# Roco-scientist/NGS-Barcode-Count

Measured on AMD Instinct MI355X. Metric: reads/sec (whole node), 3x8nt DEL vs 3x1k refs, higher is better.
Workload: dtype u8

## Files before the change

### ngs-barcode-count_amd/csrc/bc_engine.hip

```cpp
#include <hip/hip_runtime.h>
#include <string.h>
#include <stdio.h>
#include <stdlib.h>
#include <unistd.h>

#include <algorithm>
#include <functional>
#include <thread>
#include <unordered_map>
#include <string>
#include <vector>

#include "../../include/barcode_count_hip.h"
#include "bc_kernel.h"
#include "bc_engine_impl.h"
#include "bc_fold.h"
#include "bc_synth.h"

extern "C" int bc_internal_table_pack_u8(const void* d_table_u32, const void* d_bits, uint64_t n, void* d_out_u8, void* d_ovf_idx_u64,
                                         void* d_ovf_val_u32, uint64_t ovf_capacity, uint64_t* n_ovf, int device_id, void* hip_stream);

namespace bc {

template <int NW, int NWW>
// ... 609 lines not shown
  if (const char* ch = getenv("BC_COUNT_LOG_HOT")) e->log_hot = atoi(ch) != 0;
  if (const char* cd = getenv("BC_COUNT_LOG_DEFER_RESET")) e->defer_reset = atoi(cd) != 0;
  if (const char* cf = getenv("BC_COUNT_LOG_FRESH")) e->fold_fresh = atoi(cf) != 0;
  if (const char* cm = getenv("BC_COUNT_LOG_MIN_READS")) e->log_min_reads = strtoull(cm, nullptr, 0);
  if (const char* cc = getenv("BC_COUNT_LOG_CHUNK")) {
    const uint64_t c = strtoull(cc, nullptr, 0) & ~63ull;
    if (c) e->log_chunk = std::min<uint64_t>(c, 1ull << 27);
  }
  if (P.lhash_vec) {
    const int rc = upload(e, e->h.lhash.data(), e->h.lhash.size() * 4, &P.lhash_a);
    if (rc) return rc;
  }
#ifdef BC_EXPERIMENT
  if (const char* pm = getenv("BC_PIPE")) e->pipe = atoi(pm) != 0;
#endif
  HIP_TRY(hipMalloc((void**)&e->d_plan, sizeof(DevPlan)));
  HIP_TRY(hipMemcpy(e->d_plan, &P, sizeof(DevPlan), hipMemcpyHostToDevice));
  for (uint32_t g = 0; g < P.n_groups; ++g) {
    const DevGroup& G = P.groups[g];
    if (G.mode != kSetDirect) continue;
    const uint32_t nq = 1u << (2 * G.len);
    hipLaunchKernelGGL(build_dtable_kernel, dim3((nq + 255) / 256), dim3(256), 0, e->stream, e->d_plan, g,
                       reinterpret_cast<uint32_t*>((uintptr_t)G.dtable_a));
    HIP_TRY(hipGetLastError());
  }
  if (P.sparse) {
    if (table_mem) {
      set_error("bc_engine_create: the plan keeps raw captures (no dense table); pass table_mem = NULL");
      return BC_ERR_INVALID;
    }
// ... 149 lines not shown
  int rc = settle_table_on(e, e->reset_stream);
  if (rc == BC_OK && !bits_stay_owed) rc = settle_bits_on(e, e->reset_stream);
  if (hipEventRecord(e->reset_join, e->reset_stream) != hipSuccess) {
    HIP_TRY(hipStreamSynchronize(e->reset_stream));
    return rc;
  }
  *join = true;
  return rc;
}

template <int NW, int NWW>
static int launch_match(bc_engine* e, const void* d_seq, const void* d_qual, const void* d_lens, const void* d_qlens, uint32_t stride,
                        uint32_t read_len, uint32_t nd, uint64_t n_reads, uint64_t trace_off, const MatchShape& s) {
  const bool use_log = log_mode_for(e, n_reads);
  const bool hot_on = !use_log || e->log_hot;
  const bool table_untouched = use_log && !hot_on && !e->h.plan.defer_search();
  const OwedPlan owed = owed_plan(e, use_log, table_untouched);
  if (owed.table == kOwedMain) {
    const int rc = settle_table_on(e, e->stream);
    if (rc != BC_OK) return rc;
  }
  if (owed.bits == kOwedMain) {
    const int rc = settle_bits_on(e, e->stream);
    if (rc != BC_OK) return rc;
  }
  const uint32_t flags = (e->pipe ? 1u : 0u) | (s.tables_generic ? 2u : 0u) | (s.hot_generic && hot_on ? 4u : 0u);
  if (s.lds + 64 > e->lds_limit) {
    set_error("read stride too large for one LDS tile");
    return BC_ERR_UNSUPPORTED;
  }
  auto kern = match_count_kernel<NW, NWW>;
  if (s.lds > 48 * 1024) HIP_TRY(hipFuncSetAttribute((const void*)kern, hipFuncAttributeMaxDynamicSharedMemorySize, (int)s.lds));
  int per_cu = 0;
  HIP_TRY(hipOccupancyMaxActiveBlocksPerMultiprocessor(&per_cu, (const void*)kern, kTPB, s.lds));
  if (per_cu < 1) per_cu = 1;
  const uint64_t resident = (uint64_t)per_cu * e->n_cus;
  const uint64_t blocks = std::min<uint64_t>((n_reads + kTPB - 1) / kTPB, resident);
  uint64_t blocks_jit = blocks;
  hipEvent_t e0 = nullptr, e1 = nullptr;
  if (e->timing) {
    HIP_TRY(hipEventCreate(&e0));
    HIP_TRY(hipEventCreate(&e1));
    HIP_TRY(hipEventRecord(e0, e->stream));
  }
  hipFunction_t jit_fn = nullptr;
  e->reads_seen += n_reads;
  if (NW <= 8 && NWW <= 4 && e->jit_mode != 0) {
    int per_cu_jit = 1;
    jit_fn = e->jit.function(e->h.plan, e->device, e->jit_mode, e->reads_seen, s, &per_cu_jit);
    if (jit_fn) blocks_jit = std::min<uint64_t>((n_reads + kTPB - 1) / kTPB, (uint64_t)per_cu_jit * e->n_cus);
  }
  if (use_log) {
    const int rc = ensure_log(e, std::min<uint64_t>(n_reads, e->log_chunk));
    if (rc != BC_OK) return rc;
  }
  const uint64_t chunk = use_log ? e->log_chunk : n_reads;
  bool join = false;
  if (use_log) {
    const int rc = fork_owed(e, owed, &join);
    if (rc != BC_OK) {
      if (join) (void)hipStreamWaitEvent(e->stream, e->reset_join, 0);
      (void)settle_owed(e);
      return rc;
    }
  }
// ... 9 lines not shown
    const uint8_t* a_seq = (const uint8_t*)d_seq + c0 * stride;
    const uint8_t* a_qual = d_qual ? (const uint8_t*)d_qual + c0 * stride : nullptr;
    const uint16_t* a_lens = d_lens ? (const uint16_t*)d_lens + c0 : nullptr;
    const uint16_t* a_qlens = d_qlens ? (const uint16_t*)d_qlens + c0 : nullptr;
    uint8_t* a_to = e->trace_outcome ? e->trace_outcome + trace_off + c0 : nullptr;
    uint64_t* a_ti = e->trace_idx ? e->trace_idx + trace_off + c0 : nullptr;
    uint32_t* a_log = use_log ? e->d_log : nullptr;
    uint64_t a_n = n_c;
    if (jit_fn) {
      uint32_t a_region = s.region;
      uint64_t a_smask = e->n_slots ? e->n_slots - 1 : 0;
      uint32_t a_flags = (e->pipe ? 1u : 0u) | (s.tables_jit ? 2u : 0u) | (s.hot_jit && hot_on ? 4u : 0u);
      void* args[] = {&a_seq, &a_qual, &a_lens, &a_qlens, &stride, &read_len, &nd, &a_n, &a_region, &e->d_table, &e->d_bits, &e->d_slots,
                      &e->d_vals, &a_smask, &e->d_counters, &a_to, &a_ti, &a_flags, &a_log};
      const uint64_t grid = std::min<uint64_t>(blocks_jit, (n_c + kTPB - 1) / kTPB);
      HIP_TRY(hipModuleLaunchKernel(jit_fn, (uint32_t)grid, 1, 1, kTPB, 1, 1, s.lds_jit, e->stream, args, nullptr));
    } else {
      const uint64_t grid = std::min<uint64_t>(blocks, (n_c + kTPB - 1) / kTPB);
      hipLaunchKernelGGL(kern, dim3((uint32_t)grid), dim3(kTPB), s.lds, e->stream, e->d_plan, a_seq, a_qual, a_lens, a_qlens, stride, read_len,
                         nd, a_n, s.region, e->d_table, e->d_bits, e->d_slots, e->d_vals, e->n_slots ? e->n_slots - 1 : 0, e->d_counters,
                         a_to, a_ti, flags, a_log);
    }
    HIP_TRY(hipGetLastError());
    if (use_log) {
      if (join) {
        HIP_TRY(hipStreamWaitEvent(e->stream, e->reset_join, 0));
        join = false;
      }
      const bool fresh = e->owed_bits;
      const int rc = fold_log(e, n_c, fresh);
      if (rc != BC_OK) return rc;
      e->owed_bits = false;
    }
  }
  if (e->d_bits) {
    e->bits_dirty = true;
    e->reads_since_fold += n_reads;
  }
  e->last_kernel = std::string(jit_fn ? "bc_jit_match_count<" : "match_count_kernel<") +
                   std::to_string(jit_fn ? s.jit.NW : NW) + "," + std::to_string(jit_fn ? s.jit.NWW : NWW) + ">";
  if (e->timing) {
    HIP_TRY(hipEventRecord(e1, e->stream));
    e->events.emplace_back(e0, e1);
  }
  return BC_OK;
}

static int ensure_long(bc_engine* e) {
  if (e->long_ready) return BC_OK;
  if (!e->long_only && !e->src_plan->lower_long(e->lh)) return BC_ERR_UNSUPPORTED;
  LongPlan& Q = e->lh.plan;
  int rc;
  if ((rc = upload(e, e->lh.const_pos.data(), e->lh.const_pos.size() * 4, &Q.const_pos_a))) return rc;
  if ((rc = upload(e, e->lh.const_chr.data(), e->lh.const_chr.size(), &Q.const_chr_a))) return rc;
  if ((rc = upload(e, e->lh.fmtn_pos.data(), e->lh.fmtn_pos.size() * 4, &Q.fmtn_pos_a))) return rc;
// ... 104 lines not shown
  const uint32_t maxlen = d_lens ? stride : read_len;
  if (maxlen > stride) {
    set_error("submit: read_len exceeds stride");
    return BC_ERR_INVALID;
  }
  const uint32_t nd = (maxlen + 3) / 4;
  HIP_TRY(hipSetDevice(e->device));
  e->table_materialized = false;
  counts_changed(e);
  {
    const int rc = set_reserve(e, n_reads);
    if (rc != BC_OK) return rc;
  }
  if (e->long_only || maxlen > 320u) return launch_long(e, d_seq, d_qual, d_lens, d_qlens, stride, read_len, n_reads, trace_off);
  const MatchShape s = match_shape(e->h.plan, e->table_entries, stride, read_len, d_lens != nullptr, e->trace_outcome != nullptr,
                                   e->lds_limit, e->pipe, e->lhash_mode);
  const int nww = s.jit.NWW;
#define BC_LAUNCH(NW_, NWW_) \
  return launch_match<NW_, NWW_>(e, d_seq, d_qual, d_lens, d_qlens, stride, read_len, nd, n_reads, trace_off, s)
  if (s.generic_nw == 4) {
    if (nww <= 1) BC_LAUNCH(4, 1);
    if (nww <= 2) BC_LAUNCH(4, 2);
    BC_LAUNCH(4, 4);
  }
  if (s.generic_nw == 8) {
    if (nww <= 2) BC_LAUNCH(8, 2);
    if (nww <= 4) BC_LAUNCH(8, 4);
    BC_LAUNCH(8, 8);
  }
  if (nww <= 4) BC_LAUNCH(10, 4);
  BC_LAUNCH(10, 10);
// ... 979 lines not shown
  HIP_TRY(hipEventRecord(e0, 0));
  hipLaunchKernelGGL(atomic_probe_kernel, dim3(blocks), dim3(256), 0, 0, (uint32_t*)d_table_u32, entries, per, 2ull, 1u);
  HIP_TRY(hipEventRecord(e1, 0));
  hipLaunchKernelGGL(atomic_probe_kernel, dim3(blocks), dim3(256), 0, 0, (uint32_t*)d_table_u32, entries, per, 2ull, 0xFFFFFFFFu);
  HIP_TRY(hipGetLastError());
  HIP_TRY(hipDeviceSynchronize());
  float ms = 0.f;
  HIP_TRY(hipEventElapsedTime(&ms, e0, e1));
  (void)hipEventDestroy(e0);
  (void)hipEventDestroy(e1);
  if (ms > 0.f) *atomics_per_s = (double)blocks * 256.0 * per / (ms * 1e-3);
  return BC_OK;
}

const char* bc_engine_kernel_name(bc_engine* e) { return e ? e->last_kernel.c_str() : ""; }

int bc_engine_count_log_folds(const bc_engine* e, uint64_t* n) {
  *n = e->log_folds;
  return BC_OK;
}

int bc_engine_gz_blocks_inflated(const bc_engine* e, uint64_t* n) {
  *n = e->gz_blocks;
  return BC_OK;
}

int bc_engine_gz_segments_inflated(const bc_engine* e, uint64_t* n) {
  *n = e->gz_segments;
  return BC_OK;
}
// ... 314 lines not shown
```

### ngs-barcode-count_amd/csrc/bc_engine_impl.h

```cpp
#ifndef BC_ENGINE_IMPL_H
#define BC_ENGINE_IMPL_H

#include <hip/hip_runtime.h>
#include <stdint.h>

#include <string>
#include <utility>
#include <vector>

#include "../../include/barcode_count_hip.h"
#include "bc_enrich.h"
#include "bc_jit.h"
#include "bc_plan.hpp"

#define HIP_TRY(expr)                                                                      \
  do {                                                                                     \
    hipError_t _e = (expr);                                                                \
    if (_e != hipSuccess) {                                                                \
      bc::set_error(std::string(#expr) + ": " + hipGetErrorString(_e));                    \
      if (_e == hipErrorOutOfMemory) (void)hipGetLastError();  \
      return _e == hipErrorOutOfMemory ? BC_ERR_NOMEM : BC_ERR_HIP;                        \
    }                                                                                      \
  } while (0)

// ... 76 lines not shown
  std::vector<float> launch_ms;
  std::vector<uint64_t> row_idx;
  std::vector<uint32_t> row_cnt;
  static constexpr int kStages = 2;
  uint8_t* pin[kStages] = {nullptr, nullptr};
  uint8_t* dev[kStages] = {nullptr, nullptr};
  hipEvent_t copied[kStages] = {nullptr, nullptr};
  hipEvent_t consumed[kStages] = {nullptr, nullptr};
  size_t stage_bytes = 0;
  uint32_t lds_limit = 0;
  uint32_t n_cus = 0;
  bc::JitKernels jit;
  uint64_t reads_seen = 0;
  int jit_mode = 1;
  std::string last_kernel;
  bool pipe = true;
  int lhash_mode = 1;
  unsigned long long* d_slots = nullptr;
  uint32_t* d_vals = nullptr;
  uint64_t n_slots = 0;
  uint32_t key_words = 1;
  uint32_t* d_ready = nullptr;
  std::vector<uint64_t> row_wide;
  uint64_t key_bound = 0;
  bool long_only = false, long_ready = false;
  bc::LongHost lh;
  bc::LongPlan* d_long = nullptr;
  const bc_plan* src_plan = nullptr;
  bool render_pool_ready = false;
  uint32_t* d_label_off = nullptr;
  uint8_t* d_label_bytes = nullptr;
// ... 28 lines not shown
```

### ngs-barcode-count_amd/csrc/bc_jit.h

```cpp
#pragma once
#include <hip/hip_runtime.h>
#include <stdint.h>

#include <atomic>
#include <map>
#include <memory>
#include <string>
#include <thread>
#include <vector>

#include "bc_plan.hpp"

namespace bc {

struct PlanSetup {
  int lhash_mode = 1;
  uint64_t n_bit_words = 0;
  uint64_t dirty_bytes = 0;
};
PlanSetup plan_setup(HostDevPlan& h, bool long_only, bool own_table);

inline int generic_nw(uint32_t maxlen) { return maxlen <= 128 ? 4 : (maxlen <= 256 ? 8 : 10); }

struct JitShape {
  int NW, NWW;
  bool lens, tables, trace;
  uint32_t stride, read_len, region;
  bool conservative = false;
  int min_waves = 3;
};

struct MatchShape {
  int generic_nw;
  uint32_t region;
  uint32_t lds, lds_jit;
  bool tables_generic, tables_jit;
  bool hot_generic, hot_jit;
  JitShape jit;
  int first_min_waves;
  uint64_t key;
};
MatchShape match_shape(const DevPlan& P, uint64_t table_entries, uint32_t stride, uint32_t read_len, bool lens, bool trace,
                       uint32_t lds_limit, bool pipe, int lhash_mode);

struct JitKernels {
  struct Jit {
    enum { kIdle = 0, kCompiling = 1, kCodeReady = 2, kLoaded = 3, kFailed = -1 };
    std::atomic<int> state{kIdle};
    std::thread worker;
    std::vector<char> code;
    std::string log;
    hipModule_t mod = nullptr;
    hipFunction_t fn = nullptr;
    int per_cu = 0;
  };
  std::map<uint64_t, std::unique_ptr<Jit>> slots;

  JitKernels() = default;
  JitKernels(const JitKernels&) = delete;
  JitKernels& operator=(const JitKernels&) = delete;
  ~JitKernels();
  hipFunction_t function(const DevPlan& plan, int device, int mode, uint64_t reads_seen, const MatchShape& s, int* per_cu);
};

}
```

### ngs-barcode-count_amd/csrc/bc_jit.hip

```cpp
#include <hip/hip_runtime.h>
#include <hip/hiprtc.h>
#include <dlfcn.h>
#include <errno.h>
#include <fcntl.h>
#include <spawn.h>
#include <stdio.h>
#include <stdlib.h>
#include <string.h>
#include <sys/stat.h>
#include <sys/wait.h>
#include <unistd.h>

#include <algorithm>

#include "../../include/barcode_count_hip.h"
#include "bc_jit.h"
#include "bc_kernel.h"

#include "bc_jit_sources.inc"

extern char** environ;

namespace bc {

// ... 72 lines not shown
#endif
  return ps;
}

static constexpr uint32_t kGfx950LdsBytes = 160u * 1024u;

static int jit_first_min_waves(int NW, uint32_t lds_per_wg, uint32_t lds_limit) {
#ifdef BC_EXPERIMENT
  if (const char* v = getenv("BC_JIT_MIN_WAVES")) return atoi(v);
#endif
  if (NW > 4) return 2;
  const int by_lds = (int)(lds_limit / (lds_per_wg + 64u));
  return std::max(3, std::min(5, by_lds));
}

MatchShape match_shape(const DevPlan& P, uint64_t table_entries, uint32_t stride, uint32_t read_len, bool lens, bool trace,
                       uint32_t lds_limit, bool pipe, int lhash_mode) {
  MatchShape s;
  const uint32_t maxlen = lens ? stride : read_len;
  s.generic_nw = generic_nw(maxlen);
  const uint32_t slack = (uint32_t)s.generic_nw * 32u + 16u + (P.L > stride ? P.L - stride : 0u);
  s.region = (64u * stride + slack + 15u) & ~15u;
  const uint32_t lds_tiles = s.region * (kTPB / 64) * ((P.quality_on && pipe) ? 2u : 1u) +
                             (P.defer_search() ? (kTPB / 64) * kQueueBytes : 0u);
  const uint32_t lds_tables = P.lhash_vec * 16u;
  const bool tables_fit = lds_tables != 0 && 2u * (lds_tiles + lds_tables + 64u) <= lds_limit;
  s.tables_generic = lhash_mode >= 2 && tables_fit;
  s.tables_jit = lhash_mode >= 1 && tables_fit;
#ifdef BC_NO_HOT
  const bool hot_ok = false;
#else
  const bool hot_ok = !P.sparse && !P.has_random && table_entries != 0 && table_entries <= 0xFFFFFFFFull;
#endif
  const uint32_t lds_generic = lds_tiles + (s.tables_generic ? lds_tables : 0u);
  const uint32_t lds_jit = lds_tiles + (s.tables_jit ? lds_tables : 0u);
  const auto hot_fits = [&](uint32_t lds) { return hot_ok && 2u * (lds + kHotBytes + 64u) <= lds_limit; };
  s.hot_generic = hot_fits(lds_generic);
  s.hot_jit = hot_fits(lds_jit);
  s.lds = lds_generic + (s.hot_generic ? kHotBytes : 0u);
  s.lds_jit = lds_jit + (s.hot_jit ? kHotBytes : 0u);
  JitShape& sh = s.jit;
  sh.NW = (int)((maxlen + 31) / 32);
  sh.NWW = maxlen >= P.L ? (int)((maxlen - P.L + 1 + 31) / 32) : 1;
  sh.lens = lens;
  sh.tables = s.tables_jit;
  sh.trace = trace;
  sh.stride = stride;
  sh.read_len = lens ? 0u : read_len;
  sh.region = s.region;
  s.first_min_waves = jit_first_min_waves(sh.NW, s.lds_jit, lds_limit);
  s.key = ((uint64_t)stride << 32) | ((uint64_t)sh.read_len << 16) |
          (uint64_t)(((sh.NW * 16 + sh.NWW) * 2 + (lens ? 1 : 0)) * 4 + (sh.tables ? 2 : 0) + (trace ? 1 : 0));
  return s;
}

static int code_scratch_bytes(const std::vector<char>& code) {
  static const char kKey[] = ".private_segment_fixed_size";
  const size_t kl = sizeof(kKey) - 1;
  if (code.size() < kl + 5) return -1;
  for (size_t i = 0; i + kl + 5 <= code.size(); ++i) {
    if (code[i] != '.' || memcmp(&code[i], kKey, kl) != 0) continue;
    const unsigned char* v = reinterpret_cast<const unsigned char*>(&code[i + kl]);
    if (v[0] < 0x80) return v[0];
    if (v[0] == 0xcc) return v[1];
    if (v[0] == 0xcd) return (v[1] << 8) | v[2];
    if (v[0] == 0xce) return (int)(((uint32_t)v[1] << 24) | (v[2] << 16) | (v[3] << 8) | v[4]);
// ... 3 lines not shown
}

static void push_flags(std::vector<std::string>& d, const char* flags) {
  std::string t;
  for (const char* c = flags;; ++c) {
    if (*c == ' ' || *c == ';' || *c == 0) {
      if (!t.empty()) d.push_back(t);
      t.clear();
      if (*c == 0) break;
    } else {
      t += *c;
    }
  }
}

static std::vector<std::string> jit_defines(int NW, int NWW, bool lens, bool tables, bool trace, uint32_t stride, uint32_t read_len,
                                            uint32_t region, bool conservative, int min_waves) {
  std::vector<std::string> d = {"-DJIT_NW=" + std::to_string(NW), "-DJIT_NWW=" + std::to_string(NWW),
                                "-DJIT_STRIDE=" + std::to_string(stride), "-DJIT_READ_LEN=" + std::to_string(lens ? 0u : read_len),
                                "-DJIT_REGION=" + std::to_string(region),
                                lens ? "-DJIT_LENS=1" : "-DJIT_LENS=0", tables ? "-DJIT_LHASH=1" : "-DJIT_LHASH=0", trace ? "-DJIT_TRACE=1" : "-DJIT_TRACE=0",
                                "-DBC_MIN_WAVES=" + std::to_string(min_waves), "-DBC_TPB=" + std::to_string(kTPB)};
#ifdef BC_PROFILE
  d.push_back("-DBC_PROFILE=1");
#endif
  if (conservative) d.push_back("-DBC_NO_STATIC_COUNT=1");
#ifdef BC_VARIANT_FLAGS
  push_flags(d, BC_VARIANT_FLAGS);
#endif
#ifdef BC_EXPERIMENT
  d.push_back("-DBC_EXPERIMENT=1");
  if (const char* extra = getenv("BC_JIT_FLAGS")) push_flags(d, extra);
#endif
  return d;
}

// ... 99 lines not shown
    }
    rc = (WIFEXITED(status) && WEXITSTATUS(status) == 0) ? 0 : 1;
  }
  std::vector<char> lg;
  if (read_file(err, lg)) log.assign(lg.begin(), lg.end());
  const bool ok = rc == 0 && read_file(out, code);
  remove(out.c_str());
  remove(err.c_str());
  if (ok) remove(in.c_str());
  return ok;
}

static bool jit_get_code(const DevPlan& P, const std::string& arch, const JitShape& sh, bool may_compile,
                         const char* store_dir, std::vector<char>& code, std::string& log) {
  const std::string src = jit_source(P);
  const std::vector<std::string> defs = jit_defines(sh.NW, sh.NWW, sh.lens, sh.tables, sh.trace, sh.stride, sh.read_len, sh.region, sh.conservative, sh.min_waves);
  std::string key = arch + "\n" + src;
  for (const auto& d : defs) key += d;
  for (int i = 0; i < 4; ++i) key += kJitHdrText[i];
  char name[64];
  snprintf(name, sizeof name, "bcjit_%016llx", (unsigned long long)fnv1a(key));
  if (const char* src_out = getenv("BC_JIT_SRC")) write_file(src_out, src.data(), src.size());
  std::vector<std::string> dirs;
  if (store_dir) dirs.push_back(store_dir);
  if (const char* c = getenv("BC_JIT_CACHE")) dirs.push_back(c);
  dirs.push_back(lib_cache_dir());
  const char* drv = getenv("BC_JIT_COMPILER");
  const std::string driver = drv ? drv : "/opt/rocm/bin/hipcc";
  const bool have_driver = driver != "rtc" && access(driver.c_str(), X_OK) == 0;
  for (const auto& d : dirs)
    if (!d.empty() && read_file(d + "/" + name + ".co", code)) return true;
// ... 84 lines not shown
    uint64_t* f[kAddrPerGroup];
    DevGroup G = plan.groups[g];
    addr_fields(G, f);
    for (int k = 0; k < kAddrPerGroup; ++k) table[g * kAddrPerGroup + k] = *f[k];
  }
  table[kMaxGroups * kAddrPerGroup] = plan.lhash_a;
  if (hipMemcpyHtoD(addr, table.data(), table.size() * sizeof(uint64_t)) != hipSuccess) {
    out.fn = nullptr;
    return false;
  }
  std::vector<char>().swap(out.code);
  return true;
}

hipFunction_t JitKernels::function(const DevPlan& plan, int device, int mode, uint64_t reads_seen, const MatchShape& s,
                                   int* per_cu) {
  const JitShape& sh = s.jit;
  const int first_mw = s.first_min_waves;
  auto& slot = slots[s.key];
  if (!slot) slot.reset(new Jit());
  Jit& j = *slot;
  typedef Jit J;
  if (j.state.load(std::memory_order_acquire) == J::kIdle) {
    const std::string arch = jit_arch(device);
    if (jit_pick_code(plan, arch, sh, first_mw, false, nullptr, j.code, j.log)) {
      j.state.store(J::kCodeReady, std::memory_order_release);
    } else if (mode == 2) {
      const bool ok = jit_pick_code(plan, arch, sh, first_mw, true, nullptr, j.code, j.log);
      if (!ok)
        fprintf(stderr, "[barcode-count] scheme-specialised kernel did not compile; using the generic kernel\n%.2000s\n",
                j.log.c_str());
// ... 6 lines not shown
      const JitShape shape = sh;
      j.worker = std::thread([jp, own, arch, shape, first_mw]() {
        const bool ok = jit_pick_code(own, arch, shape, first_mw, true, nullptr, jp->code, jp->log);
        jp->state.store(ok ? J::kCodeReady : J::kFailed, std::memory_order_release);
      });
    } else {
      j.state.store(J::kFailed, std::memory_order_release);
    }
  }
  if (j.state.load(std::memory_order_acquire) == J::kCodeReady) {
    if (j.worker.joinable()) j.worker.join();
    bool ok = jit_load(plan, j);
    if (!ok) fprintf(stderr, "[barcode-count] using the generic kernel\n");
    if (ok && (hipModuleOccupancyMaxActiveBlocksPerMultiprocessor(&j.per_cu, j.fn, kTPB, s.lds_jit) != hipSuccess || j.per_cu < 1))
      j.per_cu = 1;
    j.state.store(ok ? J::kLoaded : J::kFailed, std::memory_order_release);
  }
  if (j.state.load(std::memory_order_acquire) == J::kFailed && j.worker.joinable()) {
    j.worker.join();
    fprintf(stderr, "[barcode-count] scheme-specialised kernel did not compile; using the generic kernel\n%.2000s\n",
            j.log.c_str());
  }
  if (j.state.load(std::memory_order_acquire) != J::kLoaded) return nullptr;
  *per_cu = j.per_cu;
  return j.fn;
}

JitKernels::~JitKernels() {
  for (auto& kv : slots) {
    if (kv.second->worker.joinable()) kv.second->worker.join();
    if (kv.second->mod) (void)hipModuleUnload(kv.second->mod);
  }
}

}

using namespace bc;

extern "C" int bc_internal_jit_compile(const bc_plan* p, uint32_t stride, uint32_t read_len, int lens, const char* cache_dir,
                                       const char* out_path) {
  if (!p) {
    set_error("bc_plan_precompile: null plan");
    return BC_ERR_INVALID;
  }
  HostDevPlan h;
  if (!p->lower(h)) return BC_ERR_UNSUPPORTED;
  const PlanSetup ps = plan_setup(h, false, true);
  const uint32_t maxlen = lens ? stride : read_len;
  if (maxlen == 0 || maxlen > stride || maxlen > 256) {
    set_error("bc_plan_precompile: read_len must be in 1..stride and at most 256 bases for a specialised kernel");
    return BC_ERR_INVALID;
  }
  const MatchShape s = match_shape(h.plan, h.plan.sparse ? 0 : h.table_entries, stride, read_len, lens != 0, false,
                                   kGfx950LdsBytes, true , ps.lhash_mode);
  std::vector<char> code;
  std::string log;
  const std::string dir = cache_dir ? cache_dir : lib_cache_dir();
  if (!jit_pick_code(h.plan, "gfx950", s.jit, s.first_min_waves, true, dir.c_str(), code, log)) {
    set_error("scheme-specialised kernel did not compile: " + log);
    return BC_ERR_INVALID;
  }
  if (out_path) write_file(out_path, code.data(), code.size());
  return BC_OK;
}

int bc_plan_precompile(const bc_plan* p, uint32_t stride, uint32_t read_len, int with_lens, const char* cache_dir) {
  return bc_internal_jit_compile(p, stride, read_len, with_lens, cache_dir, nullptr);
}
```

### ngs-barcode-count_amd/csrc/bc_kernel.h

```cpp
#pragma once
#include "bc_lane.h"

#ifdef BC_PROFILE
extern "C" __device__ unsigned long long bc_g_profile[16];
#endif

namespace bc {

#ifndef BC_TPB
#define BC_TPB 256
#endif
constexpr int kTPB = BC_TPB;
#ifndef BC_MIN_WAVES
#define BC_MIN_WAVES 3
#endif

__device__ __forceinline__ uint32_t lane_now() {
  uint32_t l;
  asm volatile("v_mbcnt_lo_u32_b32 %0, -1, 0\n\tv_mbcnt_hi_u32_b32 %0, -1, %0" : "=v"(l));
  return l;
}
__device__ __forceinline__ uint32_t wave_min_u32(uint32_t v) {
#pragma unroll
  for (int o = 32; o > 0; o >>= 1) {
// ... 443 lines not shown
  bool with_tables;
  __device__ __forceinline__ const Quad* lhash() const { return area; }
#ifdef JIT_LHASH
  __device__ __forceinline__ bool tables() const { return JIT_LHASH != 0; }
#else
  __device__ __forceinline__ bool tables() const { return with_tables; }
#endif
  uint8_t* tile;
  uint8_t* qtile;
  const uint8_t* qsrc;
  const uint8_t* next_seq;
  uint32_t bytes, region, lane;
  uint32_t chunks;
  uint32_t pending_add;
  bool qual_async;

  __device__ __forceinline__ bool any(bool c) const { return __any(c) != 0; }
  uint32_t abl_;
  bool defer_;
  __device__ __forceinline__ void issued() const { asm volatile("" ::: "memory"); }
  __device__ __forceinline__ void sequence_consumed() const {
    wave_lds_fence();
    if (next_seq) dma_tile(tile, next_seq, 64u * (bytes_per_read()), lane);
  }
  __device__ __forceinline__ uint32_t bytes_per_read() const { return stride_; }
  uint32_t stride_;
  __device__ __forceinline__ const uint32_t* stage_quality(uint32_t younger) const {
    if (qual_async) {
      wait_vm_keep((next_seq ? chunks : 0u) + pending_add + younger);
      wave_lds_fence();
      return reinterpret_cast<const uint32_t*>(qtile);
    }
    wave_lds_fence();
    stage_tile(qtile, qsrc, bytes, region, (uint8_t)'I', lane);
    wave_lds_fence();
    return reinterpret_cast<const uint32_t*>(qtile);
  }
  __device__ __forceinline__ uint32_t tier_single_n(const DevGroup& G, uint32_t q1, uint32_t q2, uint32_t qn, bool want,
                                                    bool& settled) const {
    const uint32_t lane = lane_now();
    uint32_t out = kFail;
    settled = false;
    unsigned long long todo = __ballot(want);
    const uint32_t blen = G.tier_blen, bm = (1u << blen) - 1u, nbk = 1u << (2u * blen);
// ... 208 lines not shown
    for (uint32_t i = tid; i < lhash_vec; i += kTPB) area[i] = image[i];
    ops.area = area;
    ops.with_tables = lhash_vec != 0u;
    ops.abl_ = pl.abl();
  }
  const bool hot = (flags & 4u) != 0u;
  const uint32_t hot_seed = blockIdx.x * 0x85EBCA6Bu;
  uint32_t* hot_tag = reinterpret_cast<uint32_t*>(reinterpret_cast<uint8_t*>(smem) + lhash_vec * 16u);
  uint32_t* hot_cnt = hot_tag + kHotSlots;
  if (hot) {
    for (uint32_t i = tid; i < kHotSlots; i += kTPB) {
      hot_tag[i] = kHotEmpty;
      hot_cnt[i] = 0u;
    }
  }
  const uint32_t two = (with_qual && pipe) ? 2u : 1u;
  ops.defer_ = queues && !(pl.abl() & 0x200000u);
  uint4* const dq = reinterpret_cast<uint4*>(reinterpret_cast<uint8_t*>(smem) + lhash_vec * 16u + (hot ? kHotBytes : 0u) + wave * kQueueBytes);
  uint32_t dq_plain = 0, dq_n = 0;
  uint32_t tile_seq = 0;
  ops.tile = reinterpret_cast<uint8_t*>(smem) + lhash_vec * 16u + (hot ? kHotBytes : 0u) + (queues ? (kTPB / 64) * kQueueBytes : 0u) +
             wave * region * two;
  ops.qtile = ops.tile + (two == 2u ? region : 0u);
  ops.region = region;
  ops.lane = lane;
  ops.stride_ = stride;
  const uint32_t full_bytes = 64u * stride;
  ops.chunks = (full_bytes + 1023u) / 1024u;
  ops.pending_add = 0;

  const uint64_t n_tiles = (n_reads + 63u) >> 6;
  const uint64_t n_full = n_reads >> 6;
  const uint64_t n_waves = (uint64_t)gridDim.x * (kTPB / 64);
  uint32_t acc_cnt[kNCounters];
#pragma unroll
  for (int k = 0; k < kNCounters; ++k) acc_cnt[k] = 0;
  for (uint32_t i = full_bytes + lane; i < region; i += 64) {
    ops.tile[i] = 'A';
    if (with_qual) ops.qtile[i] = 'I';
  }
  const bool logm = count_log != nullptr;
  uint32_t first_old = 0, first_on = 0, direct_tiles = 0;
  uint64_t first_idx = 0;
  uint64_t t = (uint64_t)blockIdx.x * (kTPB / 64) + wave;
  bool seq_ready = false, qual_ready = false;
  if (t < n_full && pipe) {
    dma_tile(ops.tile, seq + (t << 6) * stride, full_bytes, lane);
    seq_ready = true;
    if (with_qual) {
      dma_tile(ops.qtile, qual + (t << 6) * stride, full_bytes, lane);
      qual_ready = true;
    }
  }
  __syncthreads();
#ifdef BC_PROFILE
  for (int k = 0; k < 12; ++k) ops.acc[k] = 0;
  ops.t_last = __builtin_readcyclecounter();
#endif
  auto hot_count = [&](bool add, uint32_t key) -> bool {
    uint32_t h = ((key ^ hot_seed) * 0x9E3779B1u) >> (32u - kHotBits);
    uint32_t tag = add ? hot_tag[h] : key ^ 1u;
#ifndef BC_HOT_ONE
    if (add && tag != key && tag != kHotEmpty) {
      h = ((key ^ hot_seed) * 0xC2B2AE35u) >> (32u - kHotBits);
// ... 7 lines not shown
    if (add && tag == key) {
      atomicAdd(&hot_cnt[h], 1u);
      add = false;
    }
    return add;
  };
  for (; t < n_tiles; t += n_waves) {
    const uint64_t wfirst = t << 6;
    const uint32_t n_w = n_reads - wfirst < 64u ? (uint32_t)(n_reads - wfirst) : 64u;
    const uint64_t goff = wfirst * stride;
    const uint64_t tn = t + n_waves;
    const bool next_full = tn < n_full && pipe;
    ops.qsrc = qual + goff;
    ops.bytes = n_w * stride;
    ops.next_seq = next_full ? seq + (tn << 6) * stride : nullptr;
    ops.qual_async = qual_ready;
    if (seq_ready) {
      wait_vm_keep((qual_ready ? ops.chunks : 0u) + ops.pending_add);
      wave_lds_fence();
    } else {
      wave_lds_fence();
      stage_tile(ops.tile, seq + goff, ops.bytes, full_bytes, (uint8_t)'A', lane);
      wave_lds_fence();
    }

    ops.mark(1);
    const bool active = lane < n_w;
    uint32_t len = 0;
    if (active) len = kLens ? (uint32_t)lens[wfirst + lane] : read_len;
    uint32_t qlen = len;
    if (kLens && qlens && active) qlen = (uint32_t)qlens[wfirst + lane];
// ... 10 lines not shown
#pragma unroll
    for (uint32_t k = 0; k < kNCounters; ++k) {
      if (k == kTotalReads) continue;
      acc_cnt[k] += (uint32_t)__popcll(__ballot(active && outcome == k));
    }
    acc_cnt[kTotalReads] += n_w;
    if (trace_outcome && active && !(queues && outcome == kPending)) {
      trace_outcome[wfirst + lane] = (uint8_t)outcome;
      trace_idx[wfirst + lane] = pl.has_random ? r.dense_idx * pl.rspace + r.rcode : r.dense_idx;
    }
    bool repeat = false;
    if (bits && !logm) repeat = first_on != 0u && ((first_old >> ((uint32_t)first_idx & 31u)) & 1u) != 0u;
    const uint64_t repeat_idx = first_idx;
    seq_ready = next_full;
    qual_ready = false;
    if (next_full && with_qual) {
      wave_lds_fence();
      dma_tile(ops.qtile, qual + (tn << 6) * stride, full_bytes, lane);
      qual_ready = true;
    }
    ops.pending_add = 0;
    if (bits && !logm) {
      const uint32_t n_rep = (uint32_t)__popcll(__ballot(repeat));
      if (n_rep) {
        if (repeat) table_add_marked(pl, table, bits, repeat_idx);
        ops.pending_add += 1u;
        if (2u * n_rep > (uint32_t)__popcll(__ballot(first_on != 0u))) direct_tiles = 16u;
      }
      if (direct_tiles) --direct_tiles;
    }
    first_on = 0u;
// ... 128 lines not shown
```

### ngs-barcode-count_amd/csrc/bc_lane.h

```cpp
#pragma once
#include "bc_device_plan.h"
#include "bc_intrin.h"

#if defined(BC_JIT_TU) && JIT_READ_LEN
#define BC_STATIC_CAND(L, NWW) ((uint32_t)JIT_READ_LEN >= (L) ? (uint32_t)JIT_READ_LEN - (L) + 1u : 0u)
#else
#define BC_STATIC_CAND(L, NWW) (32u * (uint32_t)(NWW))
#endif

namespace bc {

template <int NW>
struct Planes {
  uint32_t p1[NW];
  uint32_t p2[NW];
  uint32_t pn[NW];
  uint32_t px[NW];
};

BC_HD uint64_t hash64(uint64_t x) {
  x ^= x >> 30;
  x *= 0xBF58476D1CE4E5B9ull;
  x ^= x >> 27;
  x *= 0x94D049BB133111EBull;
// ... 856 lines not shown
      res = si;
    } else if (sb == best) {
      total += sc;
    }
  }
  settled = best <= 1u;
  return (settled && total == 1u && best <= G.max_err) ? res : kFail;
}

struct ReadResult {
  uint32_t outcome;
  uint64_t dense_idx;
  uint64_t rcode;
};

template <class Ops, int NW, int NWW, bool kAligned = false>
BC_HD ReadResult process_read(const DevPlan& pl, Ops& ops, const uint32_t* seq32, uint32_t base, uint32_t len,
                              uint32_t qlen, uint32_t nd, bool active) {
  ReadResult res;
  res.outcome = kMatched;
  res.dense_idx = 0;
  res.rcode = 0;

  Planes<NW> P;
  uint32_t bad;
  if (pl.abl() & 0x40u) {
    bad = 0;
#pragma unroll
    for (int w = 0; w < NW; ++w) { P.p1[w] = base * 2654435761u + w; P.p2[w] = base * 40503u + w; P.pn[w] = 0; P.px[w] = 0; }
  } else {
// ... 65 lines not shown
          low = low || (evaluated && sum < pl.run_thr[r]);
        }
      }
      if (outcome == kMatched && low) outcome = kLowQuality;
    }
    ops.mark(5);
  };

  if (!found) start = 0;
  shr_lane<NW>(P.p1, start);
  shr_lane<NW>(P.p2, start);
  shr_lane<NW>(P.pn, start);
  if (anyx) shr_lane<NW>(P.px, start);
  uint64_t didx = 0;
  bool raw_foreign = false;
  const bool located = active && outcome == kMatched;
  const uint32_t ng = (pl.abl() & 0x20u) ? 0u : pl.n_groups;
  for (uint32_t g0 = 0; g0 < ng; g0 += 4) {
    uint32_t q1[4], q2[4], qn[4], qx[4], r[4], tl[4];
    uint32_t need_m = 0, gather_m = 0, gather_n_m = 0;
    uint32_t pend_n = 0;
#pragma unroll
    for (int u = 0; u < 4; ++u) {
      r[u] = kFail;
      tl[u] = kFail;
      q1[u] = q2[u] = qn[u] = qx[u] = 0;
      if (g0 + u < ng) {
        const DevGroup& G = pl.groups[g0 + u];
        extract_planes<NW>(P, G.off, G.len, q1[u], q2[u], qn[u]);
        if (anyx) qx[u] = extract_uniform<NW>(P.px, G.off, G.len);
// ... 150 lines not shown
            s_len = me ? G.len : s_len;
            s_max = me ? G.max_err : s_max;
            s_tab = me ? (uint64_t)G.dtable() : s_tab;
          }
        }
        uint32_t rs = kFail;
        if (pend_g) rs = single_n_lookup(reinterpret_cast<const BC_GLOBAL uint32_t*>(s_tab), s_len, s_max, s_q1, s_q2, s_qn);
#pragma unroll
        for (int u = 0; u < 4; ++u) r[u] = (pend_g != 0u && u_sel == (uint32_t)u) ? rs : r[u];
        pend_g &= pend_g - 1u;
      }
    }
#pragma unroll
    for (int u = 0; u < 4; ++u)
      if ((gather_m >> u) & 1u) r[u] = (tv[u] & 0xFFFFu) == (uint32_t)kFail16 ? kFail : (tv[u] & 0xFFFFu);
    ops.mark(7);
    const bool pre_ok = active && outcome == kMatched;
#pragma unroll
    for (int u = 0; u < 4; ++u) {
      if (g0 + u < ng) {
        const DevGroup& G = pl.groups[g0 + u];
        if (G.mode != kSetNone) {
          bool nd_ = ((need_m >> u) & 1u) && outcome == kMatched;
          if (pl.abl() & 0x2u) nd_ = false;
          if ((pl.abl() & 0x8000u) && qn[u]) nd_ = false;
          const uint32_t rr = ops.nearest(G, q1[u], q2[u], qn[u], qx[u], nd_);
          if (nd_) r[u] = rr;
          if (pre_ok && outcome == kMatched) {
            if (r[u] == kFail)
              outcome = (G.type == kGroupSample) ? kSampleBarcode : kBarcode;
            else if (pl.defer_search() && r[u] == kDeferred) {
              outcome = kPending;
              didx = (uint64_t)q1[u] | ((uint64_t)q2[u] << 32);
              pending_n = qn[u];
            } else
              didx += (uint64_t)r[u] * G.table_stride;
          }
        } else if (pre_ok && outcome == kMatched) {
          if (qx[u]) raw_foreign = true;
          didx += base5_code(q1[u], q2[u], qn[u], G.len) * G.table_stride;
        }
      }
    }
  }
  if (!quality_done) quality_filter(0u);
  if (raw_foreign && outcome == kMatched) unsupported = true;
  if (pl.has_random) {
    uint32_t r1, r2, rn;
    extract_planes<NW>(P, pl.rnd_off, pl.rnd_len, r1, r2, rn);
    const uint32_t rx = anyx ? extract_uniform<NW>(P.px, pl.rnd_off, pl.rnd_len) : 0u;
    if (rx && active && outcome == kMatched) unsupported = true;
    res.rcode = base5_code(r1, r2, rn, pl.rnd_len);
  }
  if (unsupported) outcome = kUnsupported;
  if (pl.defer_search() && outcome == kPending) res.rcode = pending_n;
  res.outcome = outcome;
  res.dense_idx = didx;
  return res;
}

// ... 2 lines not shown
```

Before: 17.82 billion.

## Share one LDS tile between sequence and quality in JIT kernel

Adds a quality-region sharing mode, on by default unless BC_QUAL_REGION=own, in which the JIT kernel stages quality bytes into the same per-wave LDS tile as the sequence instead of a separate tile. The quality DMA is issued once the sequence is consumed, and the next sequence prefetch once quality is consumed. This roughly halves tile LDS, aiming for higher occupancy. The cost is serialised DMA stages and less overlap between loads and compute. Occupancy and LDS size are also computed separately for the cold (no hot-table) path, and some launch introspection is added.

```diff
diff --git a/ngs-barcode-count_amd/csrc/bc_engine.hip b/ngs-barcode-count_amd/csrc/bc_engine.hip
--- a/ngs-barcode-count_amd/csrc/bc_engine.hip
+++ b/ngs-barcode-count_amd/csrc/bc_engine.hip
@@ -647,6 +647,7 @@
 #ifdef BC_EXPERIMENT
   if (const char* pm = getenv("BC_PIPE")) e->pipe = atoi(pm) != 0;
 #endif
+  e->qshare = qual_region_shared();
   HIP_TRY(hipMalloc((void**)&e->d_plan, sizeof(DevPlan)));
   HIP_TRY(hipMemcpy(e->d_plan, &P, sizeof(DevPlan), hipMemcpyHostToDevice));
   for (uint32_t g = 0; g < P.n_groups; ++g) {
@@ -826,6 +827,7 @@
                         uint32_t read_len, uint32_t nd, uint64_t n_reads, uint64_t trace_off, const MatchShape& s) {
   const bool use_log = log_mode_for(e, n_reads);
   const bool hot_on = !use_log || e->log_hot;
+  const uint32_t lds = hot_on ? s.lds : s.lds_cold, lds_jit = hot_on ? s.lds_jit : s.lds_jit_cold;
   const bool table_untouched = use_log && !hot_on && !e->h.plan.defer_search();
   const OwedPlan owed = owed_plan(e, use_log, table_untouched);
   if (owed.table == kOwedMain) {
@@ -844,11 +846,11 @@
   auto kern = match_count_kernel<NW, NWW>;
   if (s.lds > 48 * 1024) HIP_TRY(hipFuncSetAttribute((const void*)kern, hipFuncAttributeMaxDynamicSharedMemorySize, (int)s.lds));
   int per_cu = 0;
-  HIP_TRY(hipOccupancyMaxActiveBlocksPerMultiprocessor(&per_cu, (const void*)kern, kTPB, s.lds));
+  HIP_TRY(hipOccupancyMaxActiveBlocksPerMultiprocessor(&per_cu, (const void*)kern, kTPB, lds));
   if (per_cu < 1) per_cu = 1;
   const uint64_t resident = (uint64_t)per_cu * e->n_cus;
   const uint64_t blocks = std::min<uint64_t>((n_reads + kTPB - 1) / kTPB, resident);
-  uint64_t blocks_jit = blocks;
+  uint64_t blocks_jit = blocks, resident_jit = resident;
   hipEvent_t e0 = nullptr, e1 = nullptr;
   if (e->timing) {
     HIP_TRY(hipEventCreate(&e0));
@@ -859,8 +861,9 @@
   e->reads_seen += n_reads;
   if (NW <= 8 && NWW <= 4 && e->jit_mode != 0) {
     int per_cu_jit = 1;
-    jit_fn = e->jit.function(e->h.plan, e->device, e->jit_mode, e->reads_seen, s, &per_cu_jit);
-    if (jit_fn) blocks_jit = std::min<uint64_t>((n_reads + kTPB - 1) / kTPB, (uint64_t)per_cu_jit * e->n_cus);
+    jit_fn = e->jit.function(e->h.plan, e->device, e->jit_mode, e->reads_seen, s, hot_on, &per_cu_jit);
+    resident_jit = (uint64_t)per_cu_jit * e->n_cus;
+    if (jit_fn) blocks_jit = std::min<uint64_t>((n_reads + kTPB - 1) / kTPB, resident_jit);
   }
   if (use_log) {
     const int rc = ensure_log(e, std::min<uint64_t>(n_reads, e->log_chunk));
@@ -900,10 +903,10 @@
       void* args[] = {&a_seq, &a_qual, &a_lens, &a_qlens, &stride, &read_len, &nd, &a_n, &a_region, &e->d_table, &e->d_bits, &e->d_slots,
                       &e->d_vals, &a_smask, &e->d_counters, &a_to, &a_ti, &a_flags, &a_log};
       const uint64_t grid = std::min<uint64_t>(blocks_jit, (n_c + kTPB - 1) / kTPB);
-      HIP_TRY(hipModuleLaunchKernel(jit_fn, (uint32_t)grid, 1, 1, kTPB, 1, 1, s.lds_jit, e->stream, args, nullptr));
+      HIP_TRY(hipModuleLaunchKernel(jit_fn, (uint32_t)grid, 1, 1, kTPB, 1, 1, lds_jit, e->stream, args, nullptr));
     } else {
       const uint64_t grid = std::min<uint64_t>(blocks, (n_c + kTPB - 1) / kTPB);
-      hipLaunchKernelGGL(kern, dim3((uint32_t)grid), dim3(kTPB), s.lds, e->stream, e->d_plan, a_seq, a_qual, a_lens, a_qlens, stride, read_len,
+      hipLaunchKernelGGL(kern, dim3((uint32_t)grid), dim3(kTPB), lds, e->stream, e->d_plan, a_seq, a_qual, a_lens, a_qlens, stride, read_len,
                          nd, a_n, s.region, e->d_table, e->d_bits, e->d_slots, e->d_vals, e->n_slots ? e->n_slots - 1 : 0, e->d_counters,
                          a_to, a_ti, flags, a_log);
     }
@@ -925,6 +928,10 @@
   }
   e->last_kernel = std::string(jit_fn ? "bc_jit_match_count<" : "match_count_kernel<") +
                    std::to_string(jit_fn ? s.jit.NW : NW) + "," + std::to_string(jit_fn ? s.jit.NWW : NWW) + ">";
+  e->last_key = jit_fn ? s.key : 0;
+  e->last_lds = jit_fn ? lds_jit : lds;
+  e->last_grid = (uint32_t)std::min<uint64_t>(jit_fn ? blocks_jit : blocks, (std::min<uint64_t>(chunk, n_reads) + kTPB - 1) / kTPB);
+  e->last_resident = (uint32_t)(jit_fn ? resident_jit : resident);
   if (e->timing) {
     HIP_TRY(hipEventRecord(e1, e->stream));
     e->events.emplace_back(e0, e1);
@@ -1059,7 +1066,7 @@
   }
   if (e->long_only || maxlen > 320u) return launch_long(e, d_seq, d_qual, d_lens, d_qlens, stride, read_len, n_reads, trace_off);
   const MatchShape s = match_shape(e->h.plan, e->table_entries, stride, read_len, d_lens != nullptr, e->trace_outcome != nullptr,
-                                   e->lds_limit, e->pipe, e->lhash_mode);
+                                   e->lds_limit, e->pipe, e->qshare, e->lhash_mode);
   const int nww = s.jit.NWW;
 #define BC_LAUNCH(NW_, NWW_) \
   return launch_match<NW_, NWW_>(e, d_seq, d_qual, d_lens, d_qlens, stride, read_len, nd, n_reads, trace_off, s)
@@ -2069,6 +2076,14 @@
 }
 
 const char* bc_engine_kernel_name(bc_engine* e) { return e ? e->last_kernel.c_str() : ""; }
+
+int bc_internal_last_launch(const bc_engine* e, uint64_t* key, uint32_t* lds_bytes, uint32_t* grid, uint32_t* resident) {
+  *key = e->last_key;
+  *lds_bytes = e->last_lds;
+  *grid = e->last_grid;
+  *resident = e->last_resident;
+  return BC_OK;
+}
 
 int bc_engine_count_log_folds(const bc_engine* e, uint64_t* n) {
   *n = e->log_folds;
diff --git a/ngs-barcode-count_amd/csrc/bc_engine_impl.h b/ngs-barcode-count_amd/csrc/bc_engine_impl.h
--- a/ngs-barcode-count_amd/csrc/bc_engine_impl.h
+++ b/ngs-barcode-count_amd/csrc/bc_engine_impl.h
@@ -114,7 +114,10 @@
   uint64_t reads_seen = 0;
   int jit_mode = 1;
   std::string last_kernel;
+  uint64_t last_key = 0;
+  uint32_t last_lds = 0, last_grid = 0, last_resident = 0;
   bool pipe = true;
+  bool qshare = true;
   int lhash_mode = 1;
   unsigned long long* d_slots = nullptr;
   uint32_t* d_vals = nullptr;
diff --git a/ngs-barcode-count_amd/csrc/bc_jit.h b/ngs-barcode-count_amd/csrc/bc_jit.h
--- a/ngs-barcode-count_amd/csrc/bc_jit.h
+++ b/ngs-barcode-count_amd/csrc/bc_jit.h
@@ -25,6 +25,7 @@
 struct JitShape {
   int NW, NWW;
   bool lens, tables, trace;
+  bool qshare = false;
   uint32_t stride, read_len, region;
   bool conservative = false;
   int min_waves = 3;
@@ -34,6 +35,7 @@
   int generic_nw;
   uint32_t region;
   uint32_t lds, lds_jit;
+  uint32_t lds_cold, lds_jit_cold;
   bool tables_generic, tables_jit;
   bool hot_generic, hot_jit;
   JitShape jit;
@@ -41,7 +43,8 @@
   uint64_t key;
 };
 MatchShape match_shape(const DevPlan& P, uint64_t table_entries, uint32_t stride, uint32_t read_len, bool lens, bool trace,
-                       uint32_t lds_limit, bool pipe, int lhash_mode);
+                       uint32_t lds_limit, bool pipe, bool qshare, int lhash_mode);
+bool qual_region_shared();
 
 struct JitKernels {
   struct Jit {
@@ -52,7 +55,7 @@
     std::string log;
     hipModule_t mod = nullptr;
     hipFunction_t fn = nullptr;
-    int per_cu = 0;
+    int per_cu = 0, per_cu_cold = 0;
   };
   std::map<uint64_t, std::unique_ptr<Jit>> slots;
 
@@ -60,7 +63,8 @@
   JitKernels(const JitKernels&) = delete;
   JitKernels& operator=(const JitKernels&) = delete;
   ~JitKernels();
-  hipFunction_t function(const DevPlan& plan, int device, int mode, uint64_t reads_seen, const MatchShape& s, int* per_cu);
+  hipFunction_t function(const DevPlan& plan, int device, int mode, uint64_t reads_seen, const MatchShape& s, bool hot_on,
+                         int* per_cu);
 };
 
 }
diff --git a/ngs-barcode-count_amd/csrc/bc_jit.hip b/ngs-barcode-count_amd/csrc/bc_jit.hip
--- a/ngs-barcode-count_amd/csrc/bc_jit.hip
+++ b/ngs-barcode-count_amd/csrc/bc_jit.hip
@@ -110,15 +110,23 @@
   return std::max(3, std::min(5, by_lds));
 }
 
+bool qual_region_shared() {
+  const char* v = getenv("BC_QUAL_REGION");
+  return !(v && strcmp(v, "own") == 0);
+}
+
 MatchShape match_shape(const DevPlan& P, uint64_t table_entries, uint32_t stride, uint32_t read_len, bool lens, bool trace,
-                       uint32_t lds_limit, bool pipe, int lhash_mode) {
+                       uint32_t lds_limit, bool pipe, bool qshare, int lhash_mode) {
   MatchShape s;
   const uint32_t maxlen = lens ? stride : read_len;
   s.generic_nw = generic_nw(maxlen);
   const uint32_t slack = (uint32_t)s.generic_nw * 32u + 16u + (P.L > stride ? P.L - stride : 0u);
   s.region = (64u * stride + slack + 15u) & ~15u;
-  const uint32_t lds_tiles = s.region * (kTPB / 64) * ((P.quality_on && pipe) ? 2u : 1u) +
-                             (P.defer_search() ? (kTPB / 64) * kQueueBytes : 0u);
+  const bool two = P.quality_on && pipe;
+  const uint32_t lds_queues = P.defer_search() ? (kTPB / 64) * kQueueBytes : 0u;
+  const uint32_t lds_tiles = s.region * (kTPB / 64) * (two ? 2u : 1u) + lds_queues;
+  const bool share = two && qshare;
+  const uint32_t lds_tiles_jit = share ? s.region * (kTPB / 64) + lds_queues : lds_tiles;
   const uint32_t lds_tables = P.lhash_vec * 16u;
   const bool tables_fit = lds_tables != 0 && 2u * (lds_tiles + lds_tables + 64u) <= lds_limit;
   s.tables_generic = lhash_mode >= 2 && tables_fit;
@@ -129,10 +137,12 @@
   const bool hot_ok = !P.sparse && !P.has_random && table_entries != 0 && table_entries <= 0xFFFFFFFFull;
 #endif
   const uint32_t lds_generic = lds_tiles + (s.tables_generic ? lds_tables : 0u);
-  const uint32_t lds_jit = lds_tiles + (s.tables_jit ? lds_tables : 0u);
+  const uint32_t lds_jit = lds_tiles_jit + (s.tables_jit ? lds_tables : 0u);
   const auto hot_fits = [&](uint32_t lds) { return hot_ok && 2u * (lds + kHotBytes + 64u) <= lds_limit; };
   s.hot_generic = hot_fits(lds_generic);
-  s.hot_jit = hot_fits(lds_jit);
+  s.hot_jit = hot_fits(lds_tiles + (s.tables_jit ? lds_tables : 0u));
+  s.lds_cold = lds_generic;
+  s.lds_jit_cold = lds_jit;
   s.lds = lds_generic + (s.hot_generic ? kHotBytes : 0u);
   s.lds_jit = lds_jit + (s.hot_jit ? kHotBytes : 0u);
   JitShape& sh = s.jit;
@@ -140,12 +150,13 @@
   sh.NWW = maxlen >= P.L ? (int)((maxlen - P.L + 1 + 31) / 32) : 1;
   sh.lens = lens;
   sh.tables = s.tables_jit;
+  sh.qshare = share;
   sh.trace = trace;
   sh.stride = stride;
   sh.read_len = lens ? 0u : read_len;
   sh.region = s.region;
-  s.first_min_waves = jit_first_min_waves(sh.NW, s.lds_jit, lds_limit);
-  s.key = ((uint64_t)stride << 32) | ((uint64_t)sh.read_len << 16) |
+  s.first_min_waves = jit_first_min_waves(sh.NW, share ? s.lds_jit_cold : s.lds_jit, lds_limit);
+  s.key = ((uint64_t)stride << 32) | ((uint64_t)sh.read_len << 16) | (share ? 1ull << 15 : 0ull) |
           (uint64_t)(((sh.NW * 16 + sh.NWW) * 2 + (lens ? 1 : 0)) * 4 + (sh.tables ? 2 : 0) + (trace ? 1 : 0));
   return s;
 }
@@ -179,12 +190,12 @@
   }
 }
 
-static std::vector<std::string> jit_defines(int NW, int NWW, bool lens, bool tables, bool trace, uint32_t stride, uint32_t read_len,
-                                            uint32_t region, bool conservative, int min_waves) {
+static std::vector<std::string> jit_defines(int NW, int NWW, bool lens, bool tables, bool qshare, bool trace, uint32_t stride,
+                                            uint32_t read_len, uint32_t region, bool conservative, int min_waves) {
   std::vector<std::string> d = {"-DJIT_NW=" + std::to_string(NW), "-DJIT_NWW=" + std::to_string(NWW),
                                 "-DJIT_STRIDE=" + std::to_string(stride), "-DJIT_READ_LEN=" + std::to_string(lens ? 0u : read_len),
                                 "-DJIT_REGION=" + std::to_string(region),
-                                lens ? "-DJIT_LENS=1" : "-DJIT_LENS=0", tables ? "-DJIT_LHASH=1" : "-DJIT_LHASH=0", trace ? "-DJIT_TRACE=1" : "-DJIT_TRACE=0",
+                                lens ? "-DJIT_LENS=1" : "-DJIT_LENS=0", tables ? "-DJIT_LHASH=1" : "-DJIT_LHASH=0", qshare ? "-DJIT_QSHARE=1" : "-DJIT_QSHARE=0", trace ? "-DJIT_TRACE=1" : "-DJIT_TRACE=0",
                                 "-DBC_MIN_WAVES=" + std::to_string(min_waves), "-DBC_TPB=" + std::to_string(kTPB)};
 #ifdef BC_PROFILE
   d.push_back("-DBC_PROFILE=1");
@@ -314,7 +325,7 @@
 static bool jit_get_code(const DevPlan& P, const std::string& arch, const JitShape& sh, bool may_compile,
                          const char* store_dir, std::vector<char>& code, std::string& log) {
   const std::string src = jit_source(P);
-  const std::vector<std::string> defs = jit_defines(sh.NW, sh.NWW, sh.lens, sh.tables, sh.trace, sh.stride, sh.read_len, sh.region, sh.conservative, sh.min_waves);
+  const std::vector<std::string> defs = jit_defines(sh.NW, sh.NWW, sh.lens, sh.tables, sh.qshare, sh.trace, sh.stride, sh.read_len, sh.region, sh.conservative, sh.min_waves);
   std::string key = arch + "\n" + src;
   for (const auto& d : defs) key += d;
   for (int i = 0; i < 4; ++i) key += kJitHdrText[i];
@@ -429,7 +440,7 @@
 }
 
 hipFunction_t JitKernels::function(const DevPlan& plan, int device, int mode, uint64_t reads_seen, const MatchShape& s,
-                                   int* per_cu) {
+                                   bool hot_on, int* per_cu) {
   const JitShape& sh = s.jit;
   const int first_mw = s.first_min_waves;
   auto& slot = slots[s.key];
@@ -466,6 +477,9 @@
     if (!ok) fprintf(stderr, "[barcode-count] using the generic kernel\n");
     if (ok && (hipModuleOccupancyMaxActiveBlocksPerMultiprocessor(&j.per_cu, j.fn, kTPB, s.lds_jit) != hipSuccess || j.per_cu < 1))
       j.per_cu = 1;
+    if (ok && (hipModuleOccupancyMaxActiveBlocksPerMultiprocessor(&j.per_cu_cold, j.fn, kTPB, s.lds_jit_cold) != hipSuccess ||
+               j.per_cu_cold < 1))
+      j.per_cu_cold = 1;
     j.state.store(ok ? J::kLoaded : J::kFailed, std::memory_order_release);
   }
   if (j.state.load(std::memory_order_acquire) == J::kFailed && j.worker.joinable()) {
@@ -474,7 +488,7 @@
             j.log.c_str());
   }
   if (j.state.load(std::memory_order_acquire) != J::kLoaded) return nullptr;
-  *per_cu = j.per_cu;
+  *per_cu = hot_on ? j.per_cu : j.per_cu_cold;
   return j.fn;
 }
 
@@ -503,8 +517,12 @@
     set_error("bc_plan_precompile: read_len must be in 1..stride and at most 256 bases for a specialised kernel");
     return BC_ERR_INVALID;
   }
+  bool pipe = true;
+#ifdef BC_EXPERIMENT
+  if (const char* pm = getenv("BC_PIPE")) pipe = atoi(pm) != 0;
+#endif
   const MatchShape s = match_shape(h.plan, h.plan.sparse ? 0 : h.table_entries, stride, read_len, lens != 0, false,
-                                   kGfx950LdsBytes, true , ps.lhash_mode);
+                                   kGfx950LdsBytes, pipe, qual_region_shared(), ps.lhash_mode);
   std::vector<char> code;
   std::string log;
   const std::string dir = cache_dir ? cache_dir : lib_cache_dir();
@@ -516,6 +534,23 @@
   return BC_OK;
 }
 
+extern "C" int bc_internal_match_shape(const bc_plan* p, uint32_t stride, uint32_t read_len, int lens, int qshare, uint64_t* key,
+                                       uint32_t* lds_hot, uint32_t* lds_cold, uint32_t* region, uint32_t* tables_bytes,
+                                       int* shared) {
+  HostDevPlan h;
+  if (!p || !p->lower(h)) return BC_ERR_UNSUPPORTED;
+  const PlanSetup ps = plan_setup(h, false, true);
+  const MatchShape s = match_shape(h.plan, h.plan.sparse ? 0 : h.table_entries, stride, read_len, lens != 0, true,
+                                   kGfx950LdsBytes, true, qshare != 0, ps.lhash_mode);
+  *key = s.key;
+  *lds_hot = s.lds_jit;
+  *lds_cold = s.lds_jit_cold;
+  *region = s.region;
+  *tables_bytes = s.tables_jit ? h.plan.lhash_vec * 16u : 0u;
+  *shared = s.jit.qshare ? 1 : 0;
+  return BC_OK;
+}
+
 int bc_plan_precompile(const bc_plan* p, uint32_t stride, uint32_t read_len, int with_lens, const char* cache_dir) {
   return bc_internal_jit_compile(p, stride, read_len, with_lens, cache_dir, nullptr);
 }
diff --git a/ngs-barcode-count_amd/csrc/bc_kernel.h b/ngs-barcode-count_amd/csrc/bc_kernel.h
--- a/ngs-barcode-count_amd/csrc/bc_kernel.h
+++ b/ngs-barcode-count_amd/csrc/bc_kernel.h
@@ -481,6 +481,7 @@
   uint32_t chunks;
   uint32_t pending_add;
   bool qual_async;
+  bool share;
 
   __device__ __forceinline__ bool any(bool c) const { return __any(c) != 0; }
   uint32_t abl_;
@@ -488,13 +489,24 @@
   __device__ __forceinline__ void issued() const { asm volatile("" ::: "memory"); }
   __device__ __forceinline__ void sequence_consumed() const {
     wave_lds_fence();
-    if (next_seq) dma_tile(tile, next_seq, 64u * (bytes_per_read()), lane);
+    if (share) {
+      if (qual_async) dma_tile(tile, qsrc, 64u * (bytes_per_read()), lane);
+    } else if (next_seq) {
+      dma_tile(tile, next_seq, 64u * (bytes_per_read()), lane);
+    }
+  }
+  __device__ __forceinline__ void quality_consumed() const {
+    if (share && next_seq) {
+      __builtin_amdgcn_sched_barrier(0);
+      wave_lds_fence();
+      dma_tile(tile, next_seq, 64u * (bytes_per_read()), lane);
+    }
   }
   __device__ __forceinline__ uint32_t bytes_per_read() const { return stride_; }
   uint32_t stride_;
   __device__ __forceinline__ const uint32_t* stage_quality(uint32_t younger) const {
     if (qual_async) {
-      wait_vm_keep((next_seq ? chunks : 0u) + pending_add + younger);
+      wait_vm_keep(share ? younger : (next_seq ? chunks : 0u) + pending_add + younger);
       wave_lds_fence();
       return reinterpret_cast<const uint32_t*>(qtile);
     }
@@ -733,7 +745,12 @@
       hot_cnt[i] = 0u;
     }
   }
-  const uint32_t two = (with_qual && pipe) ? 2u : 1u;
+#ifdef JIT_QSHARE
+  const bool share = JIT_QSHARE != 0 && with_qual;
+#else
+  const bool share = false;
+#endif
+  const uint32_t two = (with_qual && pipe && !share) ? 2u : 1u;
   ops.defer_ = queues && !(pl.abl() & 0x200000u);
   uint4* const dq = reinterpret_cast<uint4*>(reinterpret_cast<uint8_t*>(smem) + lhash_vec * 16u + (hot ? kHotBytes : 0u) + wave * kQueueBytes);
   uint32_t dq_plain = 0, dq_n = 0;
@@ -741,6 +758,7 @@
   ops.tile = reinterpret_cast<uint8_t*>(smem) + lhash_vec * 16u + (hot ? kHotBytes : 0u) + (queues ? (kTPB / 64) * kQueueBytes : 0u) +
              wave * region * two;
   ops.qtile = ops.tile + (two == 2u ? region : 0u);
+  ops.share = share;
   ops.region = region;
   ops.lane = lane;
   ops.stride_ = stride;
@@ -756,7 +774,7 @@
   for (int k = 0; k < kNCounters; ++k) acc_cnt[k] = 0;
   for (uint32_t i = full_bytes + lane; i < region; i += 64) {
     ops.tile[i] = 'A';
-    if (with_qual) ops.qtile[i] = 'I';
+    if (with_qual && !share) ops.qtile[i] = 'I';
   }
   const bool logm = count_log != nullptr;
   uint32_t first_old = 0, first_on = 0, direct_tiles = 0;
@@ -766,7 +784,7 @@
   if (t < n_full && pipe) {
     dma_tile(ops.tile, seq + (t << 6) * stride, full_bytes, lane);
     seq_ready = true;
-    if (with_qual) {
+    if (with_qual && !share) {
       dma_tile(ops.qtile, qual + (t << 6) * stride, full_bytes, lane);
       qual_ready = true;
     }
@@ -804,7 +822,7 @@
     ops.qsrc = qual + goff;
     ops.bytes = n_w * stride;
     ops.next_seq = next_full ? seq + (tn << 6) * stride : nullptr;
-    ops.qual_async = qual_ready;
+    ops.qual_async = share ? seq_ready : qual_ready;
     if (seq_ready) {
       wait_vm_keep((qual_ready ? ops.chunks : 0u) + ops.pending_add);
       wave_lds_fence();
@@ -845,7 +863,7 @@
     const uint64_t repeat_idx = first_idx;
     seq_ready = next_full;
     qual_ready = false;
-    if (next_full && with_qual) {
+    if (next_full && with_qual && !share) {
       wave_lds_fence();
       dma_tile(ops.qtile, qual + (tn << 6) * stride, full_bytes, lane);
       qual_ready = true;
diff --git a/ngs-barcode-count_amd/csrc/bc_lane.h b/ngs-barcode-count_amd/csrc/bc_lane.h
--- a/ngs-barcode-count_amd/csrc/bc_lane.h
+++ b/ngs-barcode-count_amd/csrc/bc_lane.h
@@ -894,6 +894,13 @@
   uint64_t rcode;
 };
 
+template <class Ops>
+BC_HD auto ops_quality_consumed(Ops& ops, int) -> decltype(ops.quality_consumed()) {
+  ops.quality_consumed();
+}
+template <class Ops>
+BC_HD void ops_quality_consumed(Ops&, long) {}
+
 template <class Ops, int NW, int NWW, bool kAligned = false>
 BC_HD ReadResult process_read(const DevPlan& pl, Ops& ops, const uint32_t* seq32, uint32_t base, uint32_t len,
                               uint32_t qlen, uint32_t nd, bool active) {
@@ -989,6 +996,7 @@
   if (anyx) shr_lane<NW>(P.px, start);
   uint64_t didx = 0;
   bool raw_foreign = false;
+  bool quality_released = false;
   const bool located = active && outcome == kMatched;
   const uint32_t ng = (pl.abl() & 0x20u) ? 0u : pl.n_groups;
   for (uint32_t g0 = 0; g0 < ng; g0 += 4) {
@@ -1169,6 +1177,10 @@
 #pragma unroll
     for (int u = 0; u < 4; ++u)
       if ((gather_m >> u) & 1u) r[u] = (tv[u] & 0xFFFFu) == (uint32_t)kFail16 ? kFail : (tv[u] & 0xFFFFu);
+    if (!quality_released) {
+      quality_released = true;
+      ops_quality_consumed(ops, 0);
+    }
     ops.mark(7);
     const bool pre_ok = active && outcome == kMatched;
 #pragma unroll
@@ -1199,6 +1211,7 @@
     }
   }
   if (!quality_done) quality_filter(0u);
+  if (!quality_released) ops_quality_consumed(ops, 0);
   if (raw_foreign && outcome == kMatched) unsupported = true;
   if (pl.has_random) {
     uint32_t r1, r2, rn;
```

New measurement: 19.29 billion (median of 6 runs). 1.08x the previous value.
